# mahfuzalhasan/WaveFormer

Hardware: AMD Instinct MI355X
Metric: 128³×4 volumes/sec fwd (1/2/4/8 MI355X) + Dice Δ vs reference (higher is better)
Workload: dtype bf16x3; 1 GPU; MultiscaleTransformer (WaveFormer encoder) forward, 128^3x4 crops; global_batch=8, per_gpu_batch=8, precision=bf16x3, parallelism=replicas x1 (no data-path collective), hip_graph=True

## Files before the change

waveformer_amd/csrc/ffn.hip:

```cpp
#include "kernels.hpp"

namespace wf {

template <typename T>
struct Store4;
template <>
struct Store4<uint16_t> {
  typedef bf16x4 vec;
  static __device__ __forceinline__ f32x4 up(vec u) {
    return f32x4{bf2f((uint16_t)u[0]), bf2f((uint16_t)u[1]), bf2f((uint16_t)u[2]),
                 bf2f((uint16_t)u[3])};
  }
  static __device__ __forceinline__ uint16_t down(float v) { return f2bf(v); }
  static __device__ __forceinline__ vec zero() { return vec{0, 0, 0, 0}; }
  static __device__ __forceinline__ void store4(uint16_t* p, f32x4 v) {
    bf16x4 o;
    o[0] = (short)f2bf(v.x);
    o[1] = (short)f2bf(v.y);
    o[2] = (short)f2bf(v.z);
    o[3] = (short)f2bf(v.w);
    *reinterpret_cast<bf16x4*>(p) = o;
  }
};
template <>
// ... 551 lines not shown
  if (!(C % 8 == 0 && hidden % 8 == 0)) return "C and hidden must be multiples of 8";
  if (!valid_prec(prec)) return "unknown precision";
  static const bool ln1_fuse = getenv("WF_FFN_LN1_FUSE") != nullptr;
  FfnSwitches sw;
  sw.whole = getenv("WF_FFN_FUSED") != nullptr;
  sw.no_dwfc = getenv("WF_FFN_NO_DWFC") != nullptr;
  sw.ln1_fuse = ln1_fuse;
  const char* why = ffn_plan(B, C, hidden, D, H, W, prec, train, sw, p);
  if (!why && p.front == FFN_FRONT_PARTIALS) {
    GemmArgs pw = pwconv_gemm_args(nullptr, nullptr, nullptr, nullptr, nullptr, nullptr, nullptr,
                                   nullptr, 0.f, nullptr, B * D * H * W, C, hidden, prec);
    pw.epi = EPI_STORE;
    ffn_plan_set_kc_chunk(p, hidden, gemm_kc_pick_nt(pw));
  }
  return why;
}

}

using namespace wf;

extern "C" int64_t wf_ccf_ffn_workspace_bytes(int64_t B, int64_t C, int64_t hidden, int64_t D,
                                              int64_t H, int64_t W, int precision) {
  return ffn_workspace(B * D * H * W, C, hidden, precision).bytes;
}

extern "C" int wf_ccf_ffn_plan(int64_t B, int64_t C, int64_t hidden, int64_t D, int64_t H,
                               int64_t W, int precision, int train, int64_t* offsets) {
  FfnPlan plan;
  if (const char* why = ffn_plan_call(B, C, hidden, D, H, W, precision, train != 0, plan))
    return fail(WF_E_SHAPE, std::string(__func__) + ": " + why);
  if (offsets) {
    const FfnWorkspace ws = ffn_workspace(B * D * H * W, C, hidden, precision);
    const int64_t o[7] = {ws.h1, ws.h2, ws.ln2_pst, ws.ln1_pst, ws.ln1_st, ws.fcs, ws.bytes};
    for (int i = 0; i < 7; ++i) offsets[i] = o[i];
  }
  return plan.front | plan.back << 8;
}

extern "C" int wf_ccf_ffn_stage(int stage, const float* xh, const float* stats,
                                const float* n2_w, const float* n2_b,
                                const uint16_t* pw_bf16x2, const float* pw_b,
                                const float* ln1_w, const float* ln1_b, float eps1,
                                const float* dw_w, const float* dw_b, const float* ln2_w,
                                const float* ln2_b, float eps2, const uint16_t* fc_bf16x2,
                                const float* fc_b, const float* branch_scale, float* out,
                                void* workspace, int64_t B, int64_t C, int64_t hidden,
                                int64_t D, int64_t H, int64_t W, int precision, void* stream) {
  const bool train = (stage & 16) != 0;
  const int which = stage & ~16;
  WF_REQUIRE(which >= 0 && which <= 3, "stage must be 0 (all), 1 (pwconv), 2 (dwconv) or 3 (fc)");
  const bool run_pw = which == 0 || which == 1, run_dw = which == 0 || which == 2,
             run_fc = which == 0 || which == 3;
  FfnPlan plan;
  if (const char* why = ffn_plan_call(B, C, hidden, D, H, W, precision, train, plan))
    return fail(WF_E_SHAPE, std::string(__func__) + ": " + why);
  WF_REQUIRE_PTR(xh);
  WF_REQUIRE_PTR(pw_bf16x2);
  WF_REQUIRE_PTR(ln1_w);
  WF_REQUIRE_PTR(ln1_b);
  WF_REQUIRE_PTR(dw_w);
  WF_REQUIRE_PTR(dw_b);
  WF_REQUIRE_PTR(ln2_w);
  WF_REQUIRE_PTR(ln2_b);
  WF_REQUIRE_PTR(fc_bf16x2);
  WF_REQUIRE_PTR(out);
  WF_REQUIRE_PTR(workspace);
  if (stats) {
    WF_REQUIRE_PTR(n2_w);
    WF_REQUIRE_PTR(n2_b);
  }
  hipStream_t s = (hipStream_t)stream;
  const int64_t M = B * D * H * W;
  const FfnWorkspace ws = ffn_workspace(M, C, hidden, precision);
  char* base = reinterpret_cast<char*>(workspace);
  void* h1 = base + ws.h1;
  void* h2 = base + ws.h2;
  float* ln2_pst = reinterpret_cast<float*>(base + ws.ln2_pst);
  float* ln1_pst = reinterpret_cast<float*>(base + ws.ln1_pst);
  float* ln1_st = reinterpret_cast<float*>(base + ws.ln1_st);
  GemmArgs pw = pwconv_gemm_args(xh, stats, n2_w, n2_b, pw_bf16x2, pw_b, ln1_w, ln1_b, eps1, h1, M,
                                 C, hidden, precision);
  int rc = 0;
  if (run_pw && plan.front != FFN_FRONT_NONE) {
    if (plan.front != FFN_FRONT_EPILOGUE) pw.epi = EPI_STORE;
    if (plan.front == FFN_FRONT_PARTIALS) pw.o_pstats = ln1_pst;
    rc = launch_gemm(pw, s, "wf_ccf_ffn_fwd(pwconv)");
    if (!rc && plan.front == FFN_FRONT_PASS)
      rc = wf_ln_act_fwd(reinterpret_cast<const float*>(h1), ln1_w, ln1_b, eps1, 1,
                         reinterpret_cast<float*>(h1), M, hidden, stream);
    if (!rc && plan.front == FFN_FRONT_PARTIALS)
      rc = launch_ln_stats_finalize(ln1_pst, plan.ln1_np, (int)(hidden / plan.ln1_np), eps1,
                                    ln1_st, M, s);
  }
  if (rc) return rc;
  if (ffn_back_fused(plan.back)) {
    if (!run_dw) return 0;
    DwFcArgs d = dwfc_args(plan.back == FFN_BACK_FUSED ? nullptr : h1, dw_w, dw_b, ln2_w, ln2_b, eps2,
                           fc_bf16x2, fc_b, xh, stats, n2_w, n2_b, branch_scale, out, B, D, H, W);
    switch (plan.back) {
      case FFN_BACK_FUSED:
        d.pw = pw_bf16x2;
        d.pw_b = pw_b;
        d.ln1_w = ln1_w;
        d.ln1_b = ln1_b;
        d.eps1 = eps1;
        return launch_ffn_fused(d, precision, s);
      case FFN_BACK_DWFC_TB4: return launch_ffn_dwfc_tb4(d, precision, s);
      case FFN_BACK_DWFC_SB: return launch_ffn_dwfc_sb(d, precision, s);
      case FFN_BACK_DWFC2_TB: return launch_ffn_dwfc2(d, precision, true, s);
      case FFN_BACK_DWFC2_KERNEL: return launch_ffn_dwfc2(d, precision, false, s);
      default:
        d.fcs = reinterpret_cast<uint16_t*>(base + ws.fcs);
        return launch_ffn_dwfc3(d, precision, s);
    }
  }
  const bool ln2_loader = plan.back == FFN_BACK_STAGED;
  if (run_dw) {
    if (ln2_loader)
      rc = launch_dwconv3d(h1, dw_w, dw_b, h2, ln2_pst, (int)B, (int)hidden, (int)D, (int)H, (int)W,
                           precision, s, nullptr,
                           plan.front == FFN_FRONT_PARTIALS ? ln1_st : nullptr, ln1_w, ln1_b);
    else
      rc = launch_dwconv_ln_gelu(h1, dw_w, dw_b, ln2_w, ln2_b, eps2, h2, (int)B, (int)hidden,
                                 (int)D, (int)H, (int)W, precision, s);
  }
  if (rc || !run_fc) return rc;
  GemmArgs f = fc_gemm_args(h2, ln2_loader ? ln2_pst : nullptr, ln2_w, ln2_b, eps2, fc_bf16x2, fc_b,
                            xh, stats, n2_w, n2_b, branch_scale, out, M, C, hidden, D * H * W,
                            precision);
  if (!train) {
    f.kpart = reinterpret_cast<float*>(h1);
    f.kpart_bytes = ws.h2 - ws.h1;
  }
  return launch_gemm(f, s, "wf_ccf_ffn_fwd(fc)");
}

extern "C" int wf_ccf_ffn_fwd(const float* xh, const float* stats, const float* n2_w,
                              const float* n2_b, const uint16_t* pw_bf16x2, const float* pw_b,
                              const float* ln1_w, const float* ln1_b, float eps1,
                              const float* dw_w, const float* dw_b, const float* ln2_w,
                              const float* ln2_b, float eps2, const uint16_t* fc_bf16x2,
                              const float* fc_b, const float* branch_scale, float* out,
                              void* workspace, int64_t B, int64_t C, int64_t hidden, int64_t D,
                              int64_t H, int64_t W, int precision, void* stream) {
  return wf_ccf_ffn_stage(0, xh, stats, n2_w, n2_b, pw_bf16x2, pw_b, ln1_w, ln1_b, eps1, dw_w,
                          dw_b, ln2_w, ln2_b, eps2, fc_bf16x2, fc_b, branch_scale, out,
                          workspace, B, C, hidden, D, H, W, precision, stream);
}

extern "C" int wf_patch_merging_fwd(const float* x, const float* ln_w, const float* ln_b,
                                    float eps, const uint16_t* red_bf16x2, int v2, float* out,
                                    int64_t B, int64_t C, int64_t D, int64_t H, int64_t W,
                                    int precision, void* stream) {
  WF_REQUIRE(B >= 1 && C % 8 == 0 && C >= 8, "C must be a positive multiple of 8");
  WF_REQUIRE(D % 2 == 0 && H % 2 == 0 && W % 2 == 0 && D >= 2 && H >= 2 && W >= 2,
             "odd sizes (the F.pad branch, wave_helper.py:180-182) are not supported");
  WF_REQUIRE(valid_prec(precision), "unknown precision");
  WF_REQUIRE_PTR(x);
  WF_REQUIRE_PTR(ln_w);
  WF_REQUIRE_PTR(ln_b);
  WF_REQUIRE_PTR(red_bf16x2);
  WF_REQUIRE_PTR(out);
  GemmArgs g{};
  g.prec = precision;
  g.a_src = x;
  g.a_bf16 = 0;
  g.a_C = (int)C;
  g.a_nseg = 8;
  g.a_map = MAP_MERGE;
  g.merge_code = v2 ? 0x76543210 : 0x71251240;
  g.mB = (int)B;
  g.mD = (int)D;
  g.mH = (int)H;
  g.mW = (int)W;
  g.a_ln = LN_COMPUTE;
  g.a_ln_w = ln_w;
  g.a_ln_b = ln_b;
  g.a_eps = eps;
  g.w = red_bf16x2;
  g.M = B * (D / 2) * (H / 2) * (W / 2);
  g.N = (int)(2 * C);
  g.K = (int)(8 * C);
  g.epi = EPI_STORE;
  g.bias = nullptr;
  g.out = out;
  g.out_bf16 = 0;
  g.ldo = 2 * C;
  if (try_launch_merge_resident(g, (hipStream_t)stream)) return check_launch("wf_patch_merging_fwd");
  return launch_gemm(g, (hipStream_t)stream, "wf_patch_merging_fwd");
}
```

waveformer_amd/csrc/ffn_dwfc3_tb.hip:

```cpp
#include "ffn_dwfc_common.hpp"

namespace wf {

namespace tb3 {
constexpr int S2 = 3;
constexpr int C = 192, HID = 768, TY = 4, TX = 4;
constexpr int PY = TY + 2, PX = TX + 2;
constexpr int NPOS = TY * TX;
constexpr int NR = 3;
constexpr int HS = HID + 8;
constexpr int H2F = NPOS * HS;
constexpr int NT = 3;
constexpr int KS = HID / 32, KH = KS / 2;
constexpr int NTW = C / 64;
constexpr int NVEC = 2 * HID + 3 * C;
constexpr size_t LDS_BYTES = (size_t)(NT * H2F + NVEC) * 4 + 16;
static_assert(LDS_BYTES <= 160 * 1024, "LDS");
static_assert(HID * 28 <= NT * H2F, "depthwise weights and bias staged in the h2 tiles");
static_assert(S2 >= 0 && S2 <= PY, "S2");
static_assert(KS % NR == 0 && KH % NR == 0, "the weight ring keeps its phase across tiles and halves");
}

template <int NPL>
__global__ __launch_bounds__(256) void dwfc3_fc_stream_kernel(const uint16_t* __restrict__ fc,
                                                               uint16_t* __restrict__ out) {
  using namespace tb3;
  const int i = blockIdx.x * 256 + threadIdx.x;
  if (i >= 4 * KS * NTW * NPL * 64) return;
  const int lane = i & 63;
  int r = i >> 6;
  const int pl = r % NPL;
  r /= NPL;
  const int t = r % NTW;
  r /= NTW;
  const int ks = r % KS, e = r / KS;
  const int l15 = lane & 15, g4 = lane >> 4;
  const uint16_t* src = fc + (size_t)pl * C * HID + (size_t)(e * (16 * NTW) + 16 * t + l15) * HID + ks * 32 + 8 * g4;
  *reinterpret_cast<bf16x8*>(out + (size_t)i * 8) = *reinterpret_cast<const bf16x8*>(src);
}

template <int P>
__global__ __launch_bounds__(1024, 1) void ffn_dwfc3_tb_kernel(DwFcArgs a) {
  using namespace tb3;
  constexpr bool SPLIT = P == PREC_SPLIT;
  __shared__ __attribute__((aligned(16))) float h2b[NT * H2F];
  __shared__ __attribute__((aligned(16))) float vecs[NVEC];
  __shared__ int simd_cnt[4];
  float* lnw = vecs;
  float* lnb = lnw + HID;
  float* fcb = lnb + HID;
  float* n2w = fcb + C;
  float* n2b = n2w + C;

  const int tid = threadIdx.x;
  const int wid = tid >> 6, lane = tid & 63;
  const int D = a.D, H = a.H, W = a.W;
  const DwFcTile tl = dwfc_tile<TY, TX>(a);
  const int b = tl.b, x0 = tl.x0, y0 = tl.y0, z0 = tl.z0, z1 = tl.z1;
  const int plane_sz = H * W;

  if (tid < 4) simd_cnt[tid] = 0;
  dwfc_stage_ln2<HID>(lnw, lnb, a, 1024);
  dwfc_stage_epi<C>(fcb, n2w, n2b, a, 1024);
  {
    constexpr int NW = HID * 27, PER = (NW + 1023) / 1024;
    float t[PER];
#pragma unroll
    for (int j = 0; j < PER; ++j) t[j] = tid + 1024 * j < NW ? a.dw_w[tid + 1024 * j] : 0.f;
    const float tb = tid < HID ? a.dw_b[tid] : 0.f;
#pragma unroll
    for (int j = 0; j < PER; ++j)
      if (tid + 1024 * j < NW) h2b[tid + 1024 * j] = t[j];
    if (tid < HID) h2b[NW + tid] = tb;
  }
  __syncthreads();
  const int role = dwfc_wave_role<4>(simd_cnt, wid, lane);
  const int dbg = ffn_dbg(a);
  auto bar = [&]() {
    asm volatile("s_waitcnt lgkmcnt(0)" ::: "memory");
    __builtin_amdgcn_s_barrier();
    asm volatile("" ::: "memory");
  };
  auto tile_buf = [&](int t) { return h2b + ((t - z0 + 6) % NT) * H2F; };

  if (role < 12) {
    const int kslot = role % 3, c = role * 64 + lane;
    float w[27];
#pragma unroll
    for (int k = 0; k < 27; ++k) w[k] = h2b[c * 27 + k];
    const float bias = h2b[HID * 27 + c];
    float acc[3][TY][TX];
#pragma unroll
    for (int s = 0; s < 3; ++s)
#pragma unroll
      for (int o = 0; o < TY; ++o)
#pragma unroll
        for (int q = 0; q < TX; ++q) acc[s][o][q] = 0.f;
    const int lrow = 2 * (2 * (role / 3) + kslot);

    const float* src = reinterpret_cast<const float*>(a.h1) + (int64_t)b * D * plane_sz * HID;
    const int64_t plane_elems = (int64_t)plane_sz * HID;
    const int plane_bytes = (int)((plane_elems + HID) * 4);
    const int c4 = 4 * c;
    int rowoff[PY], okmask = 0;
#pragma unroll
    for (int r = 0; r < PY; ++r) {
      const int yy = y0 - 1 + r;
      rowoff[r] = (min(max(yy, 0), H - 1) * W + x0) * (HID * 4);
      if (yy >= 0 && yy < H) okmask |= 1 << r;
    }
#pragma unroll
    for (int k = 0; k < PX; ++k) {
      const int xx = x0 - 1 + k;
      if (xx >= 0 && xx < W) okmask |= 1 << (8 + k);
    }
    struct PlaneSel {
      const float* base;
      int mk;
    };
    auto plane_sel = [&](int p) {
      PlaneSel s;
// ... 145 lines not shown
  auto load_resid = [&](int z) {
    const int g = gpos0 + min(max(z, 0), D - 1) * plane_sz;
#pragma unroll
    for (int t = 0; t < NTW; ++t)
      xr[t] = __builtin_bit_cast(
          f32x4, __builtin_amdgcn_raw_buffer_load_b128(xrsrc, (g * C + col0 + 16 * t) * 4, 0, 0));
    es = __builtin_bit_cast(f32x2, __builtin_amdgcn_raw_buffer_load_b64(srsrc, g * 8, 0, 0));
  };
  f32x4 acc[NTW];
  bf16x8 ah, al;
  auto lds8 = [](const uint16_t* q) { return *reinterpret_cast<const bf16x8*>(q); };
  auto fc_half = [&](int z, auto HALFc) {
    constexpr int HALF = decltype(HALFc)::value;
    const uint16_t* Bh = reinterpret_cast<const uint16_t*>(tile_buf(z)) + (size_t)l15 * (2 * HS) + 8 * g4;
    if (HALF == 0) {
#pragma unroll
      for (int t = 0; t < NTW; ++t) acc[t] = f32x4{0.f, 0.f, 0.f, 0.f};
      ah = lds8(Bh);
      al = SPLIT ? lds8(Bh + HID) : z8;
    }
#pragma unroll
    for (int i = 0; i < KH; ++i) {
      const int ks = HALF * KH + i;
      wload(ks + 2);
      __builtin_amdgcn_sched_barrier(0);
#pragma unroll
      for (int t = 0; t < NTW; ++t) acc[t] = mma3<P>(acc[t], wh[ks % NR][t], wl[ks % NR][t], ah, al);
      __builtin_amdgcn_sched_barrier(0);
      if (ks + 1 < KS) {
        ah = lds8(Bh + (ks + 1) * 32);
        al = SPLIT ? lds8(Bh + HID + (ks + 1) * 32) : z8;
      }
    }
  };
  auto finish = [&](int z) {
#pragma unroll
    for (int t = 0; t < NTW; ++t) {
      const int col = col0 + 16 * t;
      const f32x4 v = dwfc_epilogue(acc[t], fcb, n2w, n2b, col, xr[t], es, bs, a.stats != nullptr);
      const int voff = rv ? ((gpos0 + z * plane_sz) * C + col) * 4 : BUF_OOR;
      __builtin_amdgcn_raw_buffer_store_b128(__builtin_bit_cast(u32x4, v), orsrc, voff, 0, 0);
    }
    load_resid(z + 1);
  };

  wload(0);
  wload(1);
  load_resid(z0);
  __syncthreads();
  if (dbg & 4) {
    for (int p = z0 - 1; p <= z1 + 1; ++p) {
      bar();
      bar();
    }
    return;
  }
  for (int p = z0 - 1; p < z0 + 3; ++p) {
    bar();
    bar();
  }
  for (int zo = z0; zo < z1; ++zo) {
    const bool more = zo < z1 - 1;
    fc_half(zo, std::integral_constant<int, 0>());
    if (more) bar();
    fc_half(zo, std::integral_constant<int, 1>());
    finish(zo);
    if (more) bar();
  }
}

int launch_ffn_dwfc3(const DwFcArgs& a, int prec, hipStream_t s) {
  using namespace tb3;
  if (prec != PREC_SPLIT && prec != PREC_FP16) return fail(WF_E_SHAPE, "ffn_dwfc3_tb: fp32 h1 only");
  if (!ffn_dwfc3_tb_fits(a.B, a.D, a.H, a.W))
    return fail(WF_E_SHAPE, "ffn_dwfc3_tb: tensor beyond the 2 GiB buffer-offset range");
  if (!a.fcs) return fail(WF_E_SHAPE, "ffn_dwfc3_tb: no workspace for the streamed fc weight");
  DwFcArgs g = a;
  const int64_t base = (int64_t)g.B * cdiv(g.H, TY) * cdiv(g.W, TX);
  int ZS = g.D;
  while (ZS > 8 && base * cdiv(g.D, ZS) < 256) ZS = (ZS + 1) / 2;
  g.ZS = ZS;
  g.dbg = ffn_dbg_env();
  const int64_t blocks = base * cdiv(g.D, ZS);
  const int nfrag = 4 * KS * NTW * 64 * (prec == PREC_SPLIT ? 2 : 1);
  if (prec == PREC_SPLIT)
    hipLaunchKernelGGL(dwfc3_fc_stream_kernel<2>, dim3(cdiv(nfrag, 256)), dim3(256), 0, s, g.fc, g.fcs);
  else
    hipLaunchKernelGGL(dwfc3_fc_stream_kernel<1>, dim3(cdiv(nfrag, 256)), dim3(256), 0, s, g.fc, g.fcs);
  void (*kern)(DwFcArgs) = prec == PREC_SPLIT ? ffn_dwfc3_tb_kernel<PREC_SPLIT>
                                              : ffn_dwfc3_tb_kernel<PREC_FP16>;
  hipLaunchKernelGGL(kern, dim3((unsigned)blocks), dim3(1024), 0, s, g);
  return check_launch("ffn_dwfc3_tb");
}

}
```

waveformer_amd/csrc/ffn_dwfc_common.hpp:

```cpp
#pragma once
#include "kernels.hpp"

namespace wf {

struct DwFcArgs {
  const void* h1;
  const float* dw_w;
  const float* dw_b;
  const float* ln2_w;
  const float* ln2_b;
  float eps2;
  const uint16_t* fc;
  const float* fc_b;
  const float* x;
  const float* stats;
  const float* n2_w;
  const float* n2_b;
  const float* bscale;
  float* out;
  int B, D, H, W, ZS;
  const uint16_t* pw;
  const float* pw_b;
  const float* ln1_w;
  const float* ln1_b;
  float eps1;
  int dbg;
  uint16_t* fcs;
};
#ifndef WF_FFN_DBG
#define WF_FFN_DBG 0
#endif
__device__ __forceinline__ int ffn_dbg(const DwFcArgs& a) { return WF_FFN_DBG ? a.dbg : 0; }
inline int ffn_dbg_env() {
  return WF_FFN_DBG && getenv("WF_FFN_DBG") ? atoi(getenv("WF_FFN_DBG")) : 0;
}

int launch_ffn_dwfc_tb4(const DwFcArgs& a, int prec, hipStream_t s);
int launch_ffn_dwfc_sb(const DwFcArgs& a, int prec, hipStream_t s);
int launch_ffn_dwfc2(const DwFcArgs& a, int prec, bool tb, hipStream_t s);
int launch_ffn_dwfc2_tb(const DwFcArgs& a, int prec, hipStream_t s);
int launch_ffn_dwfc3(const DwFcArgs& a, int prec, hipStream_t s);
int launch_ffn_fused(const DwFcArgs& a, int prec, hipStream_t s);

template <typename T>
struct H1Load;
template <>
struct H1Load<float> {
  typedef f32x4 raw;
  static __device__ __forceinline__ raw load(const float* p, int64_t i) {
    return *reinterpret_cast<const f32x4*>(p + i);
  }
  static __device__ __forceinline__ f32x4 up(raw u) { return u; }
};
template <>
struct H1Load<uint16_t> {
  typedef bf16x4 raw;
  static __device__ __forceinline__ raw load(const uint16_t* p, int64_t i) {
    return *reinterpret_cast<const bf16x4*>(p + i);
  }
  static __device__ __forceinline__ f32x4 up(raw u) {
    return f32x4{bf2f((uint16_t)u[0]), bf2f((uint16_t)u[1]), bf2f((uint16_t)u[2]),
                 bf2f((uint16_t)u[3])};
  }
};

#ifdef WF_DWFC2_PROBE
#define PROBE_DECL                                                              \
  const bool probe_on = blockIdx.x == 0;                                         \
  long long pr_acc[8] = {0, 0, 0, 0, 0, 0, 0, 0}, pr_last = __builtin_amdgcn_s_memtime();
#define PROBE(i)                                                                \
  if (probe_on) {                                                               \
    const long long t_ = __builtin_amdgcn_s_memtime();                          \
    pr_acc[i] += t_ - pr_last;                                                  \
    pr_last = t_;                                                               \
  }
#define PROBE_DUMP_TO(arr)                                                      \
  if (probe_on && (tid & 63) == 0)                                              \
    for (int i_ = 0; i_ < 8; ++i_) arr[wid * 8 + i_] = pr_acc[i_];
#else
#define PROBE_DECL
#define PROBE(i)
#define PROBE_DUMP_TO(arr)
#endif

constexpr int BUF_OOR = (int)0x80000000;
__device__ __forceinline__ __amdgpu_buffer_rsrc_t buf_rsrc(const void* p, int bytes) {
  return __builtin_amdgcn_make_buffer_rsrc(const_cast<void*>(p), 0, bytes, 0x00020000);
}

struct DwFcTile {
  int b, x0, y0, z0, z1;
};
template <int TY, int TX>
__device__ __forceinline__ DwFcTile dwfc_tile(const DwFcArgs& a) {
  const int ntx = (a.W + TX - 1) / TX, nty = (a.H + TY - 1) / TY, nzs = (a.D + a.ZS - 1) / a.ZS;
  int t = xcd_block_id();
  const int xt = t % ntx;
  t /= ntx;
  const int yt = t % nty;
  t /= nty;
  const int zt = t % nzs;
  DwFcTile o;
  o.b = t / nzs;
  o.x0 = xt * TX;
  o.y0 = yt * TY;
  o.z0 = zt * a.ZS;
  o.z1 = min(o.z0 + a.ZS, a.D);
  return o;
}

__device__ __forceinline__ int tb_simd_id() {
  return (int)((__builtin_amdgcn_s_getreg((1 << 11) | (4 << 6) | 4)) & 3);
}
template <int WPS>
__device__ __forceinline__ int dwfc_wave_role(int* simd_cnt, int wid, int lane) {
  const int simd = tb_simd_id();
  int slot = 0;
  if (lane == 0) slot = atomicAdd(&simd_cnt[simd], 1);
  slot = __builtin_amdgcn_readfirstlane(__shfl(slot, 0, 64));
  __syncthreads();
  const bool even = simd_cnt[0] == WPS && simd_cnt[1] == WPS && simd_cnt[2] == WPS && simd_cnt[3] == WPS;
  const int role = even ? (slot < WPS - 1 ? (WPS - 1) * simd + slot : 4 * (WPS - 1) + simd) : wid;
  return __builtin_amdgcn_readfirstlane(role);
}
// ... 74 lines not shown
```

waveformer_amd/csrc/ffn_plan.hpp:

```cpp
#pragma once
#include <stdint.h>

namespace wf {

constexpr int kFfnPrecBf16 = 0;
constexpr bool ffn_store32(int prec) { return prec != kFfnPrecBf16; }
constexpr int DW_STAT_GROUP = 32;
constexpr int64_t DWFC3_FCS_BYTES = 2 * 192 * 768 * 2;

struct FfnWorkspace {
  int64_t h1;
  int64_t h2;
  int64_t ln2_pst;
  int64_t ln1_pst;
  int64_t ln1_st;
  int64_t fcs;
  int64_t bytes;
};
inline int64_t ffn_align256(int64_t b) { return (b + 255) & ~(int64_t)255; }
inline bool ffn_has_fcs(int64_t C, int64_t hidden, int prec) {
  return C == 192 && hidden == 768 && ffn_store32(prec);
}
inline FfnWorkspace ffn_workspace(int64_t M, int64_t C, int64_t hidden, int prec) {
  const int64_t one = ffn_align256(M * hidden * (ffn_store32(prec) ? 4 : 2));
  const int64_t st = ffn_align256(M * (hidden / DW_STAT_GROUP) * 2 * 4);
  FfnWorkspace w;
  w.h1 = 0;
  w.h2 = one;
  w.ln2_pst = 2 * one;
  w.ln1_pst = w.ln2_pst + st;
  w.ln1_st = w.ln1_pst + st;
  const int64_t end = w.ln1_st + ffn_align256(M * 2 * 4);
  const bool fcs = ffn_has_fcs(C, hidden, prec);
  w.fcs = fcs ? end : -1;
  w.bytes = end + (fcs ? DWFC3_FCS_BYTES : 0);
  return w;
}

inline bool gemm_lnw_wide_shape(int64_t N, int64_t K) { return N == 768 && (K + 31) / 32 == 6; }
inline bool ffn_dwfc_tb4_fits(int64_t B, int64_t D, int64_t H, int64_t W) {
  return B * D * H * W * 48 * 4 < ((int64_t)1 << 31) && H * W * 192 * 4 < ((int64_t)1 << 31);
}
inline bool ffn_dwfc2_tb_fits(int64_t B, int64_t D, int64_t H, int64_t W) {
  return B * D * H * W * 96 * 4 < ((int64_t)1 << 31) && (H * W + 8) * 384 * 4 < ((int64_t)1 << 31);
}
inline bool ffn_dwfc3_tb_fits(int64_t B, int64_t D, int64_t H, int64_t W) {
  return B * D * H * W * 192 * 4 < ((int64_t)1 << 31) && (H * W + 8) * 768 * 4 < ((int64_t)1 << 31);
}

enum FfnFront {
  FFN_FRONT_EPILOGUE = 0,
  FFN_FRONT_PASS = 1,
  FFN_FRONT_PARTIALS = 2,
  FFN_FRONT_NONE = 3,
};
enum FfnBack {
  FFN_BACK_FUSED = 0,
  FFN_BACK_DWFC_TB4 = 1,
  FFN_BACK_DWFC_SB = 2,
  FFN_BACK_DWFC2_TB = 3,
  FFN_BACK_DWFC2_KERNEL = 4,
  FFN_BACK_DWFC3_TB = 5,
  FFN_BACK_STAGED = 6,
  FFN_BACK_STAGED_DWLN = 7,
};
struct FfnSwitches {
  bool whole;
  bool no_dwfc;
  bool ln1_fuse;
};
struct FfnPlan {
  int front, back;
  int ln1_np;
};
inline bool ffn_back_fused(int back) { return back <= FFN_BACK_DWFC3_TB; }

inline const char* ffn_plan(int64_t B, int64_t C, int64_t hidden, int64_t D, int64_t H, int64_t W,
                            int prec, bool train, const FfnSwitches& sw, FfnPlan& p) {
  const bool s32 = ffn_store32(prec);
  p.ln1_np = 0;
  if (!train && sw.whole && C == 48 && hidden == 192) {
    p.front = FFN_FRONT_NONE;
    p.back = FFN_BACK_FUSED;
    return nullptr;
  }
  const bool split_ln1 = s32 && hidden >= 768 && hidden <= 1536 && !gemm_lnw_wide_shape(hidden, C);
  p.front = !split_ln1 ? FFN_FRONT_EPILOGUE
            : !train && sw.ln1_fuse && hidden % DW_STAT_GROUP == 0 ? FFN_FRONT_PARTIALS
                                                                  : FFN_FRONT_PASS;
  if (!train && !sw.no_dwfc) {
    if (C == 48 && hidden == 192) {
      p.back = s32 && ffn_dwfc_tb4_fits(B, D, H, W) ? FFN_BACK_DWFC_TB4 : FFN_BACK_DWFC_SB;
      return nullptr;
    }
    if (C == 96 && hidden == 384) {
      p.back = s32 && ffn_dwfc2_tb_fits(B, D, H, W) ? FFN_BACK_DWFC2_TB : FFN_BACK_DWFC2_KERNEL;
      return nullptr;
    }
    if (ffn_has_fcs(C, hidden, prec) && ffn_dwfc3_tb_fits(B, D, H, W)) {
      p.back = FFN_BACK_DWFC3_TB;
      return nullptr;
    }
  }
  p.back = hidden % DW_STAT_GROUP == 0 ? FFN_BACK_STAGED : FFN_BACK_STAGED_DWLN;
  if (train && p.back != FFN_BACK_STAGED)
    return "training needs hidden % 32 == 0 (h2 kept pre-LayerNorm)";
  return nullptr;
}

inline void ffn_plan_set_kc_chunk(FfnPlan& p, int64_t hidden, int nt) {
  if (p.front != FFN_FRONT_PARTIALS) return;
  if (nt > 0 && hidden % (16 * nt) == 0) p.ln1_np = (int)(hidden / (16 * nt));
  else p.front = FFN_FRONT_PASS;
}

}
```

waveformer_amd/csrc/gemm_lnw.hip:

```cpp
#include "gemm_common.hpp"

namespace wf {

template <int NWV> struct LnwBounds { static constexpr int MINW = NWV == 4 ? 2 : 1; };
template <int P, int KS, int LW_NTW, int LW_RT, int NWV = 4>
__global__ __launch_bounds__(NWV * 64, LnwBounds<NWV>::MINW) void gemm_lnw_kernel(GemmArgs g) {
  constexpr int NTH = NWV * 64;
  constexpr int LW_N = NWV * LW_NTW * 16;
  constexpr bool SPLIT = P == PREC_SPLIT;
  constexpr int NPL = SPLIT ? 2 : 1;
  constexpr int K32 = KS * 32;
  constexpr int AS = K32 + WF_LDS_KPAD;
  constexpr int ROWS = LW_RT * 16;
  __shared__ __attribute__((aligned(16))) uint16_t As[NPL * ROWS * AS];
  __shared__ float red[NWV][ROWS];
  const int K = g.K, N = LW_N;
  const int64_t M = g.M;
  const int tid = threadIdx.x, lane = tid & 63, wid = tid >> 6;
  const int l15 = lane & 15, g4 = lane >> 4;
  const int64_t r0 = (int64_t)blockIdx.x * ROWS;
  const int cw = wid * LW_NTW * 16;

  const uint16_t* wbase = g.w + (int64_t)(cw + l15) * K + 8 * g4;
  bf16x8 wh[LW_NTW], wl[LW_NTW];
// ... 36 lines not shown
  for (int t = 0; t < LW_NTW; ++t) wload(0, t, wh[t], wl[t]);

  f32x4 acc[LW_RT][LW_NTW];
#pragma unroll
  for (int rt = 0; rt < LW_RT; ++rt)
#pragma unroll
    for (int t = 0; t < LW_NTW; ++t) acc[rt][t] = f32x4{0.f, 0.f, 0.f, 0.f};

#pragma unroll
  for (int ks = 0; ks < KS; ++ks) {
    bf16x8 ah[LW_RT], al[LW_RT];
#pragma unroll
    for (int rt = 0; rt < LW_RT; ++rt) {
      const uint16_t* p = As + (rt * 16 + l15) * AS + ks * 32 + 8 * g4;
      ah[rt] = *reinterpret_cast<const bf16x8*>(p);
      al[rt] = SPLIT ? *reinterpret_cast<const bf16x8*>(p + ROWS * AS) : z8;
    }
#pragma unroll
    for (int t = 0; t < LW_NTW; ++t) {
      const bf16x8 bh = wh[t], bl = wl[t];
#pragma unroll
      for (int rt = 0; rt < LW_RT; ++rt) acc[rt][t] = mma3<P>(acc[rt][t], bh, bl, ah[rt], al[rt]);
      __builtin_amdgcn_sched_barrier(0);
      if (t > 0 && ks + 1 < KS) wload(ks + 1, t - 1, wh[t - 1], wl[t - 1]);
      if (t == LW_NTW - 1 && ks + 1 < KS) {
        __builtin_amdgcn_sched_barrier(0);
        wload(ks + 1, t, wh[t], wl[t]);
      }
    }
  }

  const float* bias = g.bias;
#pragma unroll
  for (int t = 0; t < LW_NTW; ++t) {
    const f32x4 b4 = bias ? *reinterpret_cast<const f32x4*>(bias + cw + 16 * t + 4 * g4)
                          : f32x4{0.f, 0.f, 0.f, 0.f};
#pragma unroll
    for (int rt = 0; rt < LW_RT; ++rt) acc[rt][t] += b4;
  }
  float mean[LW_RT], rstd[LW_RT];
#pragma unroll
  for (int rt = 0; rt < LW_RT; ++rt) {
    const float s = tile_sum<LW_NTW>(acc[rt]);
    if (g4 == 0) red[wid][rt * 16 + l15] = s;
  }
  __syncthreads();
  auto wsum = [&](int r) {
    float t = (red[0][r] + red[1][r]) + (red[2][r] + red[3][r]);
#pragma unroll
    for (int w = 4; w < NWV; w += 4) t += (red[w][r] + red[w + 1][r]) + (red[w + 2][r] + red[w + 3][r]);
    return t;
  };
#pragma unroll
  for (int rt = 0; rt < LW_RT; ++rt) {
    const int r = rt * 16 + l15;
    mean[rt] = wsum(r) * (1.f / LW_N);
  }
  __syncthreads();
#pragma unroll
  for (int rt = 0; rt < LW_RT; ++rt) {
    const float q = tile_sqdev<LW_NTW>(acc[rt], mean[rt]);
    if (g4 == 0) red[wid][rt * 16 + l15] = q;
  }
  __syncthreads();
#pragma unroll
  for (int rt = 0; rt < LW_RT; ++rt) {
    const int r = rt * 16 + l15;
    rstd[rt] = rsqrtf(wsum(r) * (1.f / LW_N) + g.e_eps);
  }
#pragma unroll
  for (int t = 0; t < LW_NTW; ++t) {
    const int col = cw + 16 * t + 4 * g4;
    const f32x4 lw = *reinterpret_cast<const f32x4*>(g.e_ln_w + col) * 0.5f;
    const f32x4 lb = *reinterpret_cast<const f32x4*>(g.e_ln_b + col) * 0.5f;
#pragma unroll
    for (int rt = 0; rt < LW_RT; ++rt) {
      const int64_t row = r0 + rt * 16 + l15;
      const f32x4 v = gelu_half4((acc[rt][t] - mean[rt]) * rstd[rt] * lw + lb);
      if (row < M) store4(g.out, g.out_bf16 != 0, row * g.ldo, col, v);
    }
  }
}

template <int KS, int NTW, int RT, int NWV = 4>
void go_lnw(const GemmArgs& g, hipStream_t s) {
  const dim3 grid((unsigned)cdiv(g.M, RT * 16));
  gemm_with_prec(g.prec, false, [&](auto P, auto) {
    hipLaunchKernelGGL((gemm_lnw_kernel<P(), KS, NTW, RT, NWV>), grid, dim3(NWV * 64), 0, s, g);
  });
}


int try_launch_gemm_lnw(const GemmArgs& g, hipStream_t s) {
  if (g.epi != EPI_LN_GELU || g.a_map != MAP_IDENTITY || g.a_bf16 || g.a_gelu ||
      !(g.a_ln == LN_NONE || g.a_ln == LN_GIVEN) || g.a_C != g.K || g.K % 8 != 0 ||
      g.M >= ((int64_t)1 << 31) || g.ldo < g.N || g.ldo % 4 != 0)
    return 0;
  if (try_launch_pw2_resident(g, s)) return 1;
  const int ks = (g.K + 31) / 32;
  if (gemm_lnw_wide_shape(g)) {
    go_lnw<6, 6, 4, 8>(g, s);
    return 1;
  }
  if (g.N == 384) {
    switch (ks) {
      case 1: go_lnw<1, 6, 4>(g, s); return 1;
      case 2: go_lnw<2, 6, 4>(g, s); return 1;
      case 3: go_lnw<3, 3, 8, 8>(g, s); return 1;
      case 4: go_lnw<4, 6, 4>(g, s); return 1;
      default: return 0;
    }
  }
  return 0;
}

}
```

waveformer_amd/csrc/kernels.hpp:

```cpp
#pragma once
#include "ffn_plan.hpp"
#include "wf_common.hpp"

namespace wf {

enum Prec { PREC_BF16 = 0, PREC_SPLIT = 1, PREC_FP16 = 2 };

typedef _Float16 f16x4 __attribute__((ext_vector_type(4)));
typedef _Float16 f16x8 __attribute__((ext_vector_type(8)));
__device__ __forceinline__ uint16_t f2h(float f) { return __builtin_bit_cast(uint16_t, (_Float16)f); }

template <int P>
__device__ __forceinline__ uint16_t op_cvt(float x) {
  if constexpr (P == PREC_FP16) return f2h(x);
  else return f2bf(x);
}
template <int P>
__device__ __forceinline__ short op_lo(float x, uint16_t hi) {
  if constexpr (P == PREC_SPLIT) return (short)f2bf(x - bf2f(hi));
  else return (short)0;
}
template <int P>
__device__ __forceinline__ f32x4 mma32(bf16x8 a, bf16x8 b, f32x4 c) {
  if constexpr (P == PREC_FP16)
// ... 44 lines not shown
}
template <int P>
__device__ __forceinline__ void split8(const float (&x)[8], bf16x8& h, bf16x8& l) {
  uint32_t hw[4], lw[4];
#pragma unroll
  for (int j = 0; j < 4; ++j) split_pair<P>(x[2 * j], x[2 * j + 1], hw[j], lw[j]);
  h = __builtin_bit_cast(bf16x8, u32x4{hw[0], hw[1], hw[2], hw[3]});
  l = __builtin_bit_cast(bf16x8, u32x4{lw[0], lw[1], lw[2], lw[3]});
}
__host__ __device__ constexpr bool store32(int p) { return p != PREC_BF16; }
inline bool valid_prec(int p) { return p == PREC_BF16 || p == PREC_SPLIT || p == PREC_FP16; }

enum RowMap { MAP_IDENTITY = 0, MAP_WINDOW = 1, MAP_MERGE = 2, MAP_LEVELS = 3 };
constexpr int WF_MAX_LEVELS = 4;
enum LnMode { LN_NONE = 0, LN_GIVEN = 1, LN_COMPUTE = 2, LN_PARTIAL = 3 };
enum EpiMode { EPI_STORE = 0, EPI_LN_GELU = 1, EPI_RESID = 2, EPI_SUBVOXEL = 3 };

struct GemmArgs {
  int prec;
  const void* a_src;
  int a_bf16;
  int a_C;
  int a_nseg;
  int a_map;
  int mB, mD, mH, mW, mws;
  int merge_code;
  int a_ln;
  const float* a_stats;
  int a_np;
  const float* a_ln_w;
  const float* a_ln_b;
  float a_eps;
  int a_gelu;
  const uint16_t* w;
  int64_t M;
  int N, K;
  int epi;
  const float* bias;
  void* out;
  int out_bf16;
  int64_t ldo;
  const float* e_ln_w;
  const float* e_ln_b;
  float e_eps;
  const float* r_x;
  const float* r_stats;
  const float* r_ln_w;
  const float* r_ln_b;
  const float* r_scale;
  int64_t rows_per_sample;
  float* o_pstats;
  float* kpart;
  int64_t kpart_bytes;
  int ksplit;
  const float* lv_src[WF_MAX_LEVELS];
  int lv_row0[WF_MAX_LEVELS];
  int lv_D[WF_MAX_LEVELS], lv_H[WF_MAX_LEVELS], lv_W[WF_MAX_LEVELS];
};

int launch_gemm(const GemmArgs& g, hipStream_t s, const char* who);
int gemm_kc_pick_nt(const GemmArgs& g);
int launch_instnorm_partial(const float* x, int64_t ldx, int64_t B, int64_t C, int64_t P,
                            double* acc, hipStream_t s);
int try_launch_gemm_rows(const GemmArgs& g, hipStream_t s, bool single_chunk_only);

int launch_attn_core(const void* qkv, const float* bias, void* out, float* lse, int64_t Bw,
                     int N, int heads, int hd, float scale, int prec, hipStream_t s,
                     int table_ws = 0, int64_t pair_windows = -1, const GemmArgs* fused = nullptr);
bool attn_tbl_pair_loop(int64_t wh);

int launch_dwconv_ln_gelu(const void* in, const float* w, const float* b, const float* ln_w,
                          const float* ln_b, float eps, void* out, int B, int Hd, int D, int H,
                          int W, int prec, hipStream_t s);
int launch_dwconv3d(const void* in, const float* w, const float* b, void* out, float* pstats,
                    int B, int Hd, int D, int H, int W, int prec, hipStream_t s,
                    double* cstats = nullptr, const float* ln1_stats = nullptr,
                    const float* ln1_w = nullptr, const float* ln1_b = nullptr, int flip = 0);
int launch_ln_stats_finalize(const float* pstats, int np, int group, float eps, float* out,
                             int64_t M, hipStream_t s);
int try_launch_gemm_kc(const GemmArgs& g, hipStream_t s);
int try_launch_merge_resident(const GemmArgs& g, hipStream_t s);
int try_launch_pw2_resident(const GemmArgs& g, hipStream_t s);
int try_launch_gemm_lnw(const GemmArgs& g, hipStream_t s);
inline bool gemm_lnw_wide_shape(const GemmArgs& g) { return gemm_lnw_wide_shape(g.N, g.K); }

}

#include "ffn_dwfc_common.hpp"
```

waveformer_amd/library.py:

```python
from __future__ import annotations

import ctypes
import weakref
from typing import List, Optional, Sequence, Tuple

import torch
from torch import Tensor

from . import _lib, ops
from .autograd import _f32, _p, _s, _scale_rows, colsum, ln_bwd, ln_fwd

DETAIL_KEYS = ops.DETAIL_KEYS
SPLIT = ops.PRECISIONS["bf16x3"]
_FFN_KEEP = 16


def _empty(x: Tensor, dtype=torch.uint8) -> Tensor:
    return x.new_empty((0,), dtype=dtype)


def _round256(n):
    return (n + 255) // 256 * 256


def attn_workspace_bytes(B, C, D1, H1, W1):
    rows = B * D1 * H1 * W1
    return _round256(rows * 3 * C * 4) + _round256(rows * C * 4)


def ffn_workspace_bytes(B, C, hidden, D, H, W):
    M = B * D * H * W
    return (2 * _round256(M * hidden * 4) + 2 * _round256(M * (hidden // 32) * 2 * 4)
            + _round256(M * 2 * 4) + (2 * 192 * 768 * 2 if (C, hidden) == (192, 768) else 0))


def _ffn_offsets(B, C, hidden, D, H, W):
    off = (ctypes.c_int64 * 7)()
    if _lib.query("wf_ccf_ffn_plan", B, C, hidden, D, H, W, SPLIT, 1, off) < 0:
        raise RuntimeError(_lib.load().wf_last_error().decode(errors="replace"))
    return list(off)


@torch.library.custom_op("waveformer::dwt3d", mutates_args=(), device_types="cuda")
def dwt3d(x: Tensor, ln_w: Optional[Tensor], ln_b: Optional[Tensor], eps: float) -> Tensor:
    return ops.dwt3d_haar(x, (ln_w, ln_b, eps) if ln_w is not None else None)


@dwt3d.register_fake
def _(x, ln_w, ln_b, eps):
    B, D, H, W, C = x.shape
    return x.new_empty((8, B, D // 2, H // 2, W // 2, C))


def _dwt3d_setup(ctx, inputs, output):
    x, ln_w, ln_b, eps = inputs
    ctx.save_for_backward(x, ln_w, ln_b)
    ctx.eps = eps


@torch.library.custom_op("waveformer::dwt3d_backward", mutates_args=(), device_types="cuda")
def dwt3d_backward(gbands: Tensor, x: Tensor, ln_w: Optional[Tensor], ln_b: Optional[Tensor],
                   eps: float) -> Tuple[Tensor, Tensor, Tensor]:
    B, D, H, W, C = x.shape
    g = gbands.contiguous()
    ptrs = [g[k].data_ptr() for k in range(8)]
    strides = []
    for k in range(8):
        strides.extend(g[k].stride())
    dx = torch.empty_like(x)
    _lib.call("wf_dwt3d_haar_bwd", (ctypes.c_void_p * 8)(*ptrs), (ctypes.c_int64 * 40)(*strides),
              dx.data_ptr(), B, C, D, H, W, _s())
    if ln_w is None:
        return dx, _empty(x, torch.float32), _empty(x, torch.float32)
    dx2, dw, db = ln_bwd(x.view(-1, C), ln_w, ln_b, eps, False, dx.view(-1, C))
    return dx2.view(B, D, H, W, C), dw, db


@dwt3d_backward.register_fake
def _(gbands, x, ln_w, ln_b, eps):
    if ln_w is None:
        return torch.empty_like(x), _empty(x, torch.float32), _empty(x, torch.float32)
    return torch.empty_like(x), torch.empty_like(ln_w), torch.empty_like(ln_b)


def _dwt3d_bwd(ctx, gbands):
    x, ln_w, ln_b = ctx.saved_tensors
    dx, dw, db = torch.ops.waveformer.dwt3d_backward(gbands, x, ln_w, ln_b, ctx.eps)
    return dx, (dw if ln_w is not None else None), (db if ln_w is not None else None), None


dwt3d.register_autograd(_dwt3d_bwd, setup_context=_dwt3d_setup)


@torch.library.custom_op("waveformer::idwt3d", mutates_args=(), device_types="cuda")
def idwt3d(ll: Tensor, details: List[Tensor]) -> Tensor:
    L = len(details) // 7
    dets = [dict(zip(DETAIL_KEYS, details[7 * l:7 * l + 7])) for l in range(L)]
    return ops.idwt3d_haar(ll, dets)


@idwt3d.register_fake
def _(ll, details):
    L = len(details) // 7
    B, C, d, h, w = ll.shape
    s = 2 ** L
    return ll.new_empty((B, C, d * s, h * s, w * s))


def _idwt3d_setup(ctx, inputs, output):
    ll, details = inputs
    ctx.L = len(details) // 7
    ctx.save_for_backward(ll)


@torch.library.custom_op("waveformer::idwt3d_backward", mutates_args=(), device_types="cuda")
def idwt3d_backward(gout: Tensor, ll: Tensor, levels: int) -> List[Tensor]:
# ... 613 lines not shown
```

Baseline: 1321 volumes/s.

## Add persistent register-resident-weight pwconv GEMM for stage-3 FFN with pre-swizzled weight stream

For the stage-3 FFN (C=192, hidden=768) path, the pwconv GEMM is replaced by a new persistent kernel. It holds the pre-swizzled pw weight fragments in registers, walks row tiles across a grid sized to the CU count, and prefetches the next A tile while it runs the LN+GELU epilogue. The fc weight swizzle kernel now also swizzles the pw weight in the same launch and runs before the pwconv, and the workspace grows to hold the extra stream. This aims to cut weight reloads from LDS/global and per-block launch overhead, at the cost of one CU-count-limited grid and heavy register pressure.

Measured after the change: 1333 volumes/s, median of 6. No clear change (+0.9%).

```diff
diff --git a/waveformer_amd/csrc/ffn.hip b/waveformer_amd/csrc/ffn.hip
--- a/waveformer_amd/csrc/ffn.hip
+++ b/waveformer_amd/csrc/ffn.hip
@@ -657,7 +657,13 @@
   GemmArgs pw = pwconv_gemm_args(xh, stats, n2_w, n2_b, pw_bf16x2, pw_b, ln1_w, ln1_b, eps1, h1, M,
                                  C, hidden, precision);
   int rc = 0;
-  if (run_pw && plan.front != FFN_FRONT_NONE) {
+  const bool streams = plan.back == FFN_BACK_DWFC3_TB;
+  uint16_t* pws = streams ? reinterpret_cast<uint16_t*>(base + ws.pws) : nullptr;
+  uint16_t* fcs = streams ? reinterpret_cast<uint16_t*>(base + ws.fcs) : nullptr;
+  if (run_pw && streams) {
+    rc = launch_ffn3_streams(fc_bf16x2, fcs, pw_bf16x2, pws, precision, s);
+    if (!rc) rc = launch_gemm_lnw_walk(pw, pws, s);
+  } else if (run_pw && plan.front != FFN_FRONT_NONE) {
     if (plan.front != FFN_FRONT_EPILOGUE) pw.epi = EPI_STORE;
     if (plan.front == FFN_FRONT_PARTIALS) pw.o_pstats = ln1_pst;
     rc = launch_gemm(pw, s, "wf_ccf_ffn_fwd(pwconv)");
@@ -686,7 +692,7 @@
       case FFN_BACK_DWFC2_TB: return launch_ffn_dwfc2(d, precision, true, s);
       case FFN_BACK_DWFC2_KERNEL: return launch_ffn_dwfc2(d, precision, false, s);
       default:
-        d.fcs = reinterpret_cast<uint16_t*>(base + ws.fcs);
+        d.fcs = fcs;
         return launch_ffn_dwfc3(d, precision, s);
     }
   }
diff --git a/waveformer_amd/csrc/ffn_dwfc3_tb.hip b/waveformer_amd/csrc/ffn_dwfc3_tb.hip
--- a/waveformer_amd/csrc/ffn_dwfc3_tb.hip
+++ b/waveformer_amd/csrc/ffn_dwfc3_tb.hip
@@ -21,22 +21,32 @@
 static_assert(KS % NR == 0 && KH % NR == 0, "the weight ring keeps its phase across tiles and halves");
 }
 
-template <int NPL>
-__global__ __launch_bounds__(256) void dwfc3_fc_stream_kernel(const uint16_t* __restrict__ fc,
-                                                               uint16_t* __restrict__ out) {
-  using namespace tb3;
-  const int i = blockIdx.x * 256 + threadIdx.x;
-  if (i >= 4 * KS * NTW * NPL * 64) return;
+template <int NPL, int WK, int WT>
+__device__ __forceinline__ void stream_fragment(const uint16_t* __restrict__ w, int ld, int i,
+                                                uint16_t* __restrict__ out) {
+  using namespace tb3;
   const int lane = i & 63;
   int r = i >> 6;
   const int pl = r % NPL;
   r /= NPL;
-  const int t = r % NTW;
-  r /= NTW;
-  const int ks = r % KS, e = r / KS;
+  const int t = r % WT;
+  r /= WT;
+  const int ks = r % WK, e = r / WK;
   const int l15 = lane & 15, g4 = lane >> 4;
-  const uint16_t* src = fc + (size_t)pl * C * HID + (size_t)(e * (16 * NTW) + 16 * t + l15) * HID + ks * 32 + 8 * g4;
+  const uint16_t* src = w + (size_t)pl * C * HID + (size_t)(e * (16 * WT) + 16 * t + l15) * ld + ks * 32 + 8 * g4;
   *reinterpret_cast<bf16x8*>(out + (size_t)i * 8) = *reinterpret_cast<const bf16x8*>(src);
+}
+template <int NPL>
+__global__ __launch_bounds__(256) void dwfc3_fc_stream_kernel(const uint16_t* __restrict__ fc,
+                                                               uint16_t* __restrict__ out,
+                                                               const uint16_t* __restrict__ pw,
+                                                               uint16_t* __restrict__ pw_out) {
+  using namespace tb3;
+  constexpr int NF = NPL * C * HID / 8;
+  static_assert(NF == 4 * KS * NTW * NPL * 64 && NF % 256 == 0, "whole workgroups per weight");
+  const int i = blockIdx.x * 256 + threadIdx.x;
+  if (i < NF) stream_fragment<NPL, KS, NTW>(fc, HID, i, out);
+  else stream_fragment<NPL, C / 32, HID / 128>(pw, C, i - NF, pw_out);
 }
 
 template <int P>
@@ -348,15 +358,23 @@
   g.ZS = ZS;
   g.dbg = ffn_dbg_env();
   const int64_t blocks = base * cdiv(g.D, ZS);
-  const int nfrag = 4 * KS * NTW * 64 * (prec == PREC_SPLIT ? 2 : 1);
-  if (prec == PREC_SPLIT)
-    hipLaunchKernelGGL(dwfc3_fc_stream_kernel<2>, dim3(cdiv(nfrag, 256)), dim3(256), 0, s, g.fc, g.fcs);
-  else
-    hipLaunchKernelGGL(dwfc3_fc_stream_kernel<1>, dim3(cdiv(nfrag, 256)), dim3(256), 0, s, g.fc, g.fcs);
   void (*kern)(DwFcArgs) = prec == PREC_SPLIT ? ffn_dwfc3_tb_kernel<PREC_SPLIT>
                                               : ffn_dwfc3_tb_kernel<PREC_FP16>;
   hipLaunchKernelGGL(kern, dim3((unsigned)blocks), dim3(1024), 0, s, g);
   return check_launch("ffn_dwfc3_tb");
 }
 
-}
+int launch_ffn3_streams(const uint16_t* fc, uint16_t* fcs, const uint16_t* pw, uint16_t* pws,
+                        int prec, hipStream_t s) {
+  using namespace tb3;
+  if (prec != PREC_SPLIT && prec != PREC_FP16) return fail(WF_E_SHAPE, "ffn3_streams: fp32 h1 only");
+  if (!fc || !fcs || (pw && !pws)) return fail(WF_E_SHAPE, "ffn3_streams: no workspace for a stream");
+  const int nfrag = (prec == PREC_SPLIT ? 2 : 1) * C * HID / 8 * (pw ? 2 : 1);
+  if (prec == PREC_SPLIT)
+    hipLaunchKernelGGL(dwfc3_fc_stream_kernel<2>, dim3(nfrag / 256), dim3(256), 0, s, fc, fcs, pw, pws);
+  else
+    hipLaunchKernelGGL(dwfc3_fc_stream_kernel<1>, dim3(nfrag / 256), dim3(256), 0, s, fc, fcs, pw, pws);
+  return check_launch("ffn3_streams");
+}
+
+}
diff --git a/waveformer_amd/csrc/ffn_dwfc_common.hpp b/waveformer_amd/csrc/ffn_dwfc_common.hpp
--- a/waveformer_amd/csrc/ffn_dwfc_common.hpp
+++ b/waveformer_amd/csrc/ffn_dwfc_common.hpp
@@ -40,6 +40,8 @@
 int launch_ffn_dwfc2(const DwFcArgs& a, int prec, bool tb, hipStream_t s);
 int launch_ffn_dwfc2_tb(const DwFcArgs& a, int prec, hipStream_t s);
 int launch_ffn_dwfc3(const DwFcArgs& a, int prec, hipStream_t s);
+int launch_ffn3_streams(const uint16_t* fc, uint16_t* fcs, const uint16_t* pw, uint16_t* pws,
+                        int prec, hipStream_t s);
 int launch_ffn_fused(const DwFcArgs& a, int prec, hipStream_t s);
 
 template <typename T>
diff --git a/waveformer_amd/csrc/ffn_plan.hpp b/waveformer_amd/csrc/ffn_plan.hpp
--- a/waveformer_amd/csrc/ffn_plan.hpp
+++ b/waveformer_amd/csrc/ffn_plan.hpp
@@ -7,6 +7,7 @@
 constexpr bool ffn_store32(int prec) { return prec != kFfnPrecBf16; }
 constexpr int DW_STAT_GROUP = 32;
 constexpr int64_t DWFC3_FCS_BYTES = 2 * 192 * 768 * 2;
+constexpr int64_t PW3_STREAM_BYTES = 2 * 768 * 192 * 2;
 
 struct FfnWorkspace {
   int64_t h1;
@@ -14,6 +15,7 @@
   int64_t ln2_pst;
   int64_t ln1_pst;
   int64_t ln1_st;
+  int64_t pws;
   int64_t fcs;
   int64_t bytes;
 };
@@ -32,8 +34,9 @@
   w.ln1_st = w.ln1_pst + st;
   const int64_t end = w.ln1_st + ffn_align256(M * 2 * 4);
   const bool fcs = ffn_has_fcs(C, hidden, prec);
-  w.fcs = fcs ? end : -1;
-  w.bytes = end + (fcs ? DWFC3_FCS_BYTES : 0);
+  w.pws = fcs ? end : -1;
+  w.fcs = fcs ? end + PW3_STREAM_BYTES : -1;
+  w.bytes = end + (fcs ? PW3_STREAM_BYTES + DWFC3_FCS_BYTES : 0);
   return w;
 }
 
diff --git a/waveformer_amd/csrc/gemm_lnw.hip b/waveformer_amd/csrc/gemm_lnw.hip
--- a/waveformer_amd/csrc/gemm_lnw.hip
+++ b/waveformer_amd/csrc/gemm_lnw.hip
@@ -142,6 +142,211 @@
   }
 }
 
+namespace lnw3 {
+constexpr int K = 192, N = 768, KS = K / 32, NWV = 8, NTW = 6, RT = 4, ROWS = RT * 16;
+constexpr int NTH = NWV * 64;
+constexpr int AS = K + WF_LDS_KPAD;
+constexpr int Q = K / 4;
+constexpr int NQ = ROWS * Q / NTH;
+static_assert(NTH == 8 * ROWS && Q == 8 * NQ && NWV * NTW * 16 == N, "tile");
+}
+
+template <int P>
+__global__ __launch_bounds__(lnw3::NTH, 1) void gemm_lnw_walk_kernel(GemmArgs g,
+                                                                     const uint16_t* __restrict__ wst,
+                                                                     int dbg_) {
+  using namespace lnw3;
+  constexpr bool SPLIT = P == PREC_SPLIT;
+  constexpr int NPL = SPLIT ? 2 : 1;
+  __shared__ __attribute__((aligned(16))) uint16_t As[NPL * ROWS * AS];
+  __shared__ float red[2][NWV][ROWS];
+  __shared__ __attribute__((aligned(16))) float alw[K], alb[K];
+  __shared__ __attribute__((aligned(16))) float ebi[N], elw[N], elb[N];
+  const int dbg = WF_FFN_DBG ? dbg_ : 0;
+  const int64_t M = g.M;
+  const int tid = threadIdx.x, lane = tid & 63, wid = tid >> 6;
+  const int l15 = lane & 15, g4 = lane >> 4;
+  const int cw = wid * NTW * 16;
+  const int ntiles = (int)((M + ROWS - 1) / ROWS);
+  const bool given = g.a_ln == LN_GIVEN;
+  auto bar = [&]() {
+    asm volatile("s_waitcnt lgkmcnt(0)" ::: "memory");
+    __builtin_amdgcn_s_barrier();
+    asm volatile("" ::: "memory");
+  };
+
+  for (int i = tid; i < N; i += NTH) {
+    ebi[i] = g.bias ? g.bias[i] : 0.f;
+    elw[i] = g.e_ln_w[i] * 0.5f;
+    elb[i] = g.e_ln_b[i] * 0.5f;
+  }
+  if (given && tid < K) {
+    alw[tid] = g.a_ln_w[tid];
+    alb[tid] = g.a_ln_b[tid];
+  }
+
+  const __amdgpu_buffer_rsrc_t wrsrc = buf_rsrc(wst, NPL * N * K * 2);
+  const int wvoff = wid * (KS * NTW * NPL * 1024) + 16 * lane;
+  bf16x8 wh[NTW], wl[NTW];
+  const bf16x8 z8 = {0, 0, 0, 0, 0, 0, 0, 0};
+  auto wload = [&](int ks, int t) {
+    const int so = (ks * NTW + t) * NPL * 1024;
+    wh[t] = __builtin_bit_cast(bf16x8, __builtin_amdgcn_raw_buffer_load_b128(wrsrc, wvoff, so, 0));
+    if (SPLIT) wl[t] = __builtin_bit_cast(bf16x8, __builtin_amdgcn_raw_buffer_load_b128(wrsrc, wvoff, so + 1024, 0));
+    else wl[t] = z8;
+  };
+
+  const int ar = tid >> 3, ac = tid & 7;
+  f32x4 av[NQ];
+  f32x2 ast = {0.f, 1.f};
+  auto fetch = [&](int tile) {
+    const int64_t row = min((int64_t)tile * ROWS + ar, M - 1);
+    const float* src = reinterpret_cast<const float*>(g.a_src) + row * K + 4 * ac;
+#pragma unroll
+    for (int j = 0; j < NQ; ++j) av[j] = *reinterpret_cast<const f32x4*>(src + 32 * j);
+    if (given) ast = *reinterpret_cast<const f32x2*>(g.a_stats + 2 * row);
+  };
+  auto commit = [&]() {
+#pragma unroll
+    for (int j = 0; j < NQ; ++j) {
+      const int k = 4 * ac + 32 * j;
+      f32x4 v = av[j];
+      if (given) {
+        const float mu = ast.x, rs = ast.y;
+        const f32x4 lw = *reinterpret_cast<const f32x4*>(alw + k);
+        const f32x4 lb = *reinterpret_cast<const f32x4*>(alb + k);
+        v = (v - mu) * rs * lw + lb;
+      }
+      bf16x4 h4, l4;
+#pragma unroll
+      for (int e = 0; e < 4; ++e) {
+        const uint16_t hb = op_cvt<P>(v[e]);
+        h4[e] = (short)hb;
+        l4[e] = op_lo<P>(v[e], hb);
+      }
+      *reinterpret_cast<bf16x4*>(As + ar * AS + k) = h4;
+      if (SPLIT) *reinterpret_cast<bf16x4*>(As + ROWS * AS + ar * AS + k) = l4;
+    }
+  };
+
+  int tile = blockIdx.x;
+#pragma unroll
+  for (int t = 0; t < NTW; ++t) wload(0, t);
+  if (!(dbg & 4)) fetch(tile);
+  bar();
+  if (!(dbg & 4)) commit();
+  bar();
+
+  for (; tile < ntiles; tile += gridDim.x) {
+    const int64_t r0 = (int64_t)tile * ROWS;
+    const bool more = tile + (int)gridDim.x < ntiles;
+    f32x4 acc[RT][NTW];
+#pragma unroll
+    for (int rt = 0; rt < RT; ++rt)
+#pragma unroll
+      for (int t = 0; t < NTW; ++t) acc[rt][t] = f32x4{0.f, 0.f, 0.f, 0.f};
+
+    if (!(dbg & 2)) {
+#pragma unroll
+      for (int ks = 0; ks < KS; ++ks) {
+        bf16x8 ah[RT], al[RT];
+#pragma unroll
+        for (int rt = 0; rt < RT; ++rt) {
+          const uint16_t* p = As + (rt * 16 + l15) * AS + ks * 32 + 8 * g4;
+          ah[rt] = *reinterpret_cast<const bf16x8*>(p);
+          al[rt] = SPLIT ? *reinterpret_cast<const bf16x8*>(p + ROWS * AS) : z8;
+        }
+#pragma unroll
+        for (int t = 0; t < NTW; ++t) {
+          const bf16x8 bh = wh[t], bl = wl[t];
+#pragma unroll
+          for (int rt = 0; rt < RT; ++rt) acc[rt][t] = mma3<P>(acc[rt][t], bh, bl, ah[rt], al[rt]);
+          __builtin_amdgcn_sched_barrier(0);
+          if (t > 0) wload((ks + 1) % KS, t - 1);
+          if (t == NTW - 1) {
+            __builtin_amdgcn_sched_barrier(0);
+            wload((ks + 1) % KS, t);
+          }
+        }
+      }
+    }
+    if (more && !(dbg & 4)) fetch(tile + (int)gridDim.x);
+    if (dbg & 1) {
+      bar();
+      if (more && !(dbg & 4)) commit();
+      bar();
+      if (acc[0][0].x == 12345.678f) store4(g.out, false, r0 * g.ldo, cw, acc[1][1] + acc[2][2] + acc[3][3]);
+      continue;
+    }
+
+#pragma unroll
+    for (int t = 0; t < NTW; ++t) {
+      const f32x4 b4 = *reinterpret_cast<const f32x4*>(ebi + cw + 16 * t + 4 * g4);
+#pragma unroll
+      for (int rt = 0; rt < RT; ++rt) acc[rt][t] += b4;
+    }
+    float mean[RT], rstd[RT];
+#pragma unroll
+    for (int rt = 0; rt < RT; ++rt) {
+      const float s = tile_sum<NTW>(acc[rt]);
+      if (g4 == 0) red[0][wid][rt * 16 + l15] = s;
+    }
+    bar();
+    auto wsum = [&](const float (*rd)[ROWS], int r) {
+      float t = (rd[0][r] + rd[1][r]) + (rd[2][r] + rd[3][r]);
+#pragma unroll
+      for (int w = 4; w < NWV; w += 4) t += (rd[w][r] + rd[w + 1][r]) + (rd[w + 2][r] + rd[w + 3][r]);
+      return t;
+    };
+#pragma unroll
+    for (int rt = 0; rt < RT; ++rt) mean[rt] = wsum(red[0], rt * 16 + l15) * (1.f / N);
+#pragma unroll
+    for (int rt = 0; rt < RT; ++rt) {
+      const float q = tile_sqdev<NTW>(acc[rt], mean[rt]);
+      if (g4 == 0) red[1][wid][rt * 16 + l15] = q;
+    }
+    if (more && !(dbg & 4)) commit();
+    bar();
+#pragma unroll
+    for (int rt = 0; rt < RT; ++rt) rstd[rt] = rsqrtf(wsum(red[1], rt * 16 + l15) * (1.f / N) + g.e_eps);
+#pragma unroll
+    for (int t = 0; t < NTW; ++t) {
+      const int col = cw + 16 * t + 4 * g4;
+      const f32x4 lw = *reinterpret_cast<const f32x4*>(elw + col);
+      const f32x4 lb = *reinterpret_cast<const f32x4*>(elb + col);
+#pragma unroll
+      for (int rt = 0; rt < RT; ++rt) {
+        const int64_t row = r0 + rt * 16 + l15;
+        const f32x4 v = gelu_half4((acc[rt][t] - mean[rt]) * rstd[rt] * lw + lb);
+        if (row < M) store4(g.out, false, row * g.ldo, col, v);
+      }
+    }
+  }
+}
+
+int launch_gemm_lnw_walk(const GemmArgs& g, const uint16_t* wstream, hipStream_t s) {
+  using namespace lnw3;
+  if (g.epi != EPI_LN_GELU || g.a_map != MAP_IDENTITY || g.a_bf16 || g.a_gelu || g.out_bf16 ||
+      !(g.a_ln == LN_NONE || g.a_ln == LN_GIVEN) || g.a_C != K || g.K != K || g.N != N ||
+      g.M < 1 || g.M >= ((int64_t)1 << 31) || g.ldo < N || g.ldo % 4 != 0 || !wstream ||
+      !(g.prec == PREC_SPLIT || g.prec == PREC_FP16))
+    return fail(WF_E_SHAPE, "gemm_lnw_walk: the stage-3 pwconv with fp32 h1 only");
+  static int cus = 0;
+  if (!cus) {
+    int dev = 0;
+    (void)hipGetDevice(&dev);
+    (void)hipDeviceGetAttribute(&cus, hipDeviceAttributeMultiprocessorCount, dev);
+    if (cus <= 0) cus = 256;
+  }
+  const int64_t tiles = cdiv(g.M, ROWS);
+  const dim3 grid((unsigned)(tiles < cus ? tiles : cus));
+  if (g.prec == PREC_SPLIT)
+    hipLaunchKernelGGL(gemm_lnw_walk_kernel<PREC_SPLIT>, grid, dim3(NTH), 0, s, g, wstream, ffn_dbg_env());
+  else
+    hipLaunchKernelGGL(gemm_lnw_walk_kernel<PREC_FP16>, grid, dim3(NTH), 0, s, g, wstream, ffn_dbg_env());
+  return check_launch("gemm_lnw_walk");
+}
+
 template <int KS, int NTW, int RT, int NWV = 4>
 void go_lnw(const GemmArgs& g, hipStream_t s) {
   const dim3 grid((unsigned)cdiv(g.M, RT * 16));
diff --git a/waveformer_amd/csrc/kernels.hpp b/waveformer_amd/csrc/kernels.hpp
--- a/waveformer_amd/csrc/kernels.hpp
+++ b/waveformer_amd/csrc/kernels.hpp
@@ -150,6 +150,7 @@
 int try_launch_merge_resident(const GemmArgs& g, hipStream_t s);
 int try_launch_pw2_resident(const GemmArgs& g, hipStream_t s);
 int try_launch_gemm_lnw(const GemmArgs& g, hipStream_t s);
+int launch_gemm_lnw_walk(const GemmArgs& g, const uint16_t* wstream, hipStream_t s);
 inline bool gemm_lnw_wide_shape(const GemmArgs& g) { return gemm_lnw_wide_shape(g.N, g.K); }
 
 }
diff --git a/waveformer_amd/library.py b/waveformer_amd/library.py
--- a/waveformer_amd/library.py
+++ b/waveformer_amd/library.py
@@ -31,7 +31,7 @@
 def ffn_workspace_bytes(B, C, hidden, D, H, W):
     M = B * D * H * W
     return (2 * _round256(M * hidden * 4) + 2 * _round256(M * (hidden // 32) * 2 * 4)
-            + _round256(M * 2 * 4) + (2 * 192 * 768 * 2 if (C, hidden) == (192, 768) else 0))
+            + _round256(M * 2 * 4) + (2 * (2 * 192 * 768 * 2) if (C, hidden) == (192, 768) else 0))
 
 
 def _ffn_offsets(B, C, hidden, D, H, W):
```
